# chlhnu/DOT-SOCP

Measured on AMD Instinct MI355X. Metric: ADMM iters/sec on NxNxT dot2d staggered grid at 1/2/4/8 MI355X, higher is better.
Workload: dtype f64

## Files before the change

### dot-socp_amd/csrc/fused.hip

```cpp
#include "device_utils.h"
#include "gather_tile.h"
#include "kernels.h"

#include <cstdlib>

namespace dotsocp {

template <int MODE, int XB, bool NT = false, bool GIN = false, bool GOUT = false>
__global__ void __launch_bounds__(64 * XB) k_cone_fused(Grid g, LoopCoef c, FusedArgs a) {
    static_assert(MODE == 1 || !(GIN || GOUT), "the gamma form exists between two MODE_B passes only");
    constexpr bool DUAL = (MODE >= 5);
    constexpr bool UPD = (MODE != 0 && MODE != 6);
    constexpr bool PROJ = (MODE < 2 || MODE >= 5);
    __shared__ double2 xch[2][XB][64];
    __shared__ double2 xchp[DUAL ? 2 : 1][DUAL ? XB : 1][DUAL ? 64 : 1];
    const int lane = threadIdx.x, xl = threadIdx.y;
    const BlockId blk = block_id(a.xcd != 0);
    const i64 y = (i64)blk.x * 64 + lane;
    const i64 x = (i64)blk.y * XB + xl;
    const bool inb = (y < g.ny) && (x < g.nx);
    const i64 yc = inb ? y : 0, xc = inb ? x : 0;
    const i64 t0 = ((i64)blk.z + a.z0) * a.TC;
    const i64 t1 = (t0 + a.TC < g.ncl) ? t0 + a.TC : g.ncl;
    const bool lastChunk = (t1 == g.ncl);
// ... 10 lines not shown
        const i64 ci = yc + g.py * xc;
        gc.p3 = a.carry_in[ci]; gc.p4 = a.carry_in[g.plane + ci];
        gc.p7 = a.carry_in[2 * g.plane + ci]; gc.p8 = a.carry_in[3 * g.plane + ci];
    }
    const i64 tstop = (GATHER && lastChunk) ? t1 + 1 : t1;
    for (i64 tl = tstart; tl < tstop; ++tl) {
        const bool hasCell = tl < g.ncl;
        const bool own = tl >= t0;
        double w[10], wp[10];
        if (hasCell) {
            const i64 i = yc + g.py * (xc + g.nx * tl);
            const EdgeQuad nxt = load_edges(g, a.q, yc, xc, tl + 1, c.sf);
            double b[10], v[10];
#pragma unroll
            for (int j = 0; j < 10; ++j) b[j] = ld_stream<NT>(a.beta_in + j * g.Nc + i);
            if (!GIN) apply_scale_ops(b, a.bops);
            build_z2(v, a.q[i], cur, nxt, c.s, c.dF);
            if constexpr (GIN) {
#pragma unroll
                for (int j = 0; j < 10; ++j) b[j] = mult_finish(b[j], v[j], c.tau);
                if (!GOUT && own && inb) {
#pragma unroll
                    for (int j = 0; j < 10; ++j) st_stream<NT>(a.beta_out + j * g.Nc + i, b[j]);
                }
            } else if constexpr (UPD) {
                const EdgeQuad nxto = load_edges(g, a.q_old, yc, xc, tl + 1, c.sf);
                double zo[10];
                build_z2(zo, a.q_old[i], curo, nxto, c.s, c.dF);
#pragma unroll
                for (int j = 0; j < 10; ++j) zo[j] = zo[j] - b[j];
                proj_row<10>(zo);
#pragma unroll
                for (int j = 0; j < 10; ++j) b[j] = mult_finish(mult_carry(b[j], zo[j], c.tau), v[j], c.tau);
                if (own && inb) {
                    if (MODE != 3 && !GOUT) {
#pragma unroll
                        for (int j = 0; j < 10; ++j) st_stream<NT>(a.beta_out + j * g.Nc + i, b[j]);
                    }
                    if (MODE == 2 || MODE == 3) {
#pragma unroll
                        for (int j = 0; j < 10; ++j) st_stream<NT>(a.z_out + j * g.Nc + i, zo[j]);
                    }
                }
                curo = nxto;
                if (MODE == 4) {
#pragma unroll
                    for (int j = 0; j < 10; ++j) w[j] = zo[j] + b[j];
                    if (own && inb) a.q2[i] = c.s * (w[9] - w[0]);
                }
            }
            cur = nxt;
            if (PROJ) {
                if (MODE == 5) {
                    const EdgeQuad nxt3 = load_edges(g, a.q3, yc, xc, tl + 1, c.sf);
                    build_z2(v, a.q3[i], cur3, nxt3, c.s, c.dF);
                    cur3 = nxt3;
                }
#pragma unroll
                for (int j = 0; j < 10; ++j) v[j] = v[j] - b[j];
                proj_row<10>(v);
                if (GOUT && own && inb) {
#pragma unroll
                    for (int j = 0; j < 10; ++j) st_stream<NT>(a.beta_out + j * g.Nc + i, mult_carry(b[j], v[j], c.tau));
                }
#pragma unroll
                for (int j = 0; j < 10; ++j) w[j] = v[j] + b[j];
// ... 106 lines not shown
```

### dot-socp_amd/csrc/kernels.h

```cpp
#pragma once
#include "common.h"
#include "defer.h"
#include "particle_block.h"

namespace dotsocp {

struct LoopCoef {
    double s;
    double sf;
    double dF;
    double at, ax, ay;
    double tau;
    double c1, c2;
    double dinv1, dinv2;
};

enum {
    S_Q2 = 0, S_Z2, S_APHI2, S_ALPHA2, S_BETA2, S_FBBETA2, S_PRIM1, S_PRIM2, S_DUAL1, S_DUAL2,
    S_COMPLEM, S_DOTCOMP, S_RHO2, S_RHOFQ2, S_MRHOB, S_M2, S_RHOB2, S_QALPHA, S_CPHI, S_PHI2,
    S_COUNT
};

struct KktCoef {
    double sigma;
// ... 15 lines not shown
        return true;
    }
};

int launch_proj_soc(double *out, const double *in, i64 M, i64 K, hipStream_t st);
int launch_bfd(const Grid &g, double *z, const double *q, double s, double dF, hipStream_t st);
int launch_bfd_conj(const Grid &g, double *q, const double *w, double s, hipStream_t st, const double *tail_bx = nullptr,
                    const double *tail_by = nullptr);
int launch_cone_proj(const Grid &g, const LoopCoef &c, const double *q, const double *beta, double *z,
                     hipStream_t st);
int launch_beta_update(const Grid &g, const LoopCoef &c, const double *q, const double *z, double *beta,
                       hipStream_t st);
int launch_gather_tail(const Grid &g, const double *z, const double *beta, double *tail_bx, double *tail_by,
                       hipStream_t st);

struct FusedGeom {
    int XB;
    i64 nyblk, nxblk;
    i64 TC, chunks;
    i64 sx_len, sy_len;
};
struct FusedArgs {
    const double *q_old;
    const double *q;
    const double *beta_in;
    double *beta_out;
    double *z_out;
    double *q2;
    double *sx, *sy;
    const double *q3;
    double *p2, *sxp, *syp;
    i64 TC;
    ScaleOps bops;
    int xcd;
    int z0;
    const double *carry_in;
    double *carry_out;
};
bool tile_xcd_remap(const Grid &g);
int fused_geometry(const Grid &g, FusedGeom &fg);
enum { CONE_GIN = 1, CONE_GOUT = 2 };
int launch_cone_fused(int mode, const Grid &g, const LoopCoef &c, const FusedGeom &fg, FusedArgs a,
                      hipStream_t st, i64 z0 = 0, i64 zcount = -1, int flavour = 0);
bool cone_split_enabled();

struct KktWork;
struct AccArgs {
    const double *q;
    const double *z_in, *beta_in;
    const double *z0, *beta0;
    double *z0_out, *beta0_out;
    double bdiv;
    KktCoef kk;
    const double *alpha_p, *weight;
    double *partials;
    int nostore;
    double *z_out, *beta_out;
    double *q2, *sx, *sy;
    i64 TC;
    double c1, c2, om_rho, rho;
};
struct AccCoef {
    double c1, c2, om_rho, rho;
    double om_c1, c1c2;
};
int launch_acc_cone(int mode, const Grid &g, const LoopCoef &c, const FusedGeom &fg, AccArgs a, hipStream_t st);
// ... 220 lines not shown
```

### dot-socp_amd/csrc/kkt.hip

```cpp
#include "device_utils.h"
#include "gather_tile.h"
#include "kernels.h"

#include <cstdlib>

namespace dotsocp {

struct WBeta {
    const double *b;
    i64 Nz;
    __device__ __forceinline__ double operator()(int j, i64 cell) const { return b[j * Nz + cell]; }
};

template <bool WEIGHTED, int PART, bool NODUAL = false>
__global__ void __launch_bounds__(TILE_Y *TILE_X) k_kkt(Grid g, LoopCoef c, KktCoef k, i64 chunk,
                                                         const double *__restrict__ phi, const double *__restrict__ q,
                                                         const double *__restrict__ alpha, const double *__restrict__ z,
                                                         const double *__restrict__ beta,
                                                         const double *__restrict__ cvec,
                                                         const double *__restrict__ weight,
                                                         KktHalo halo, double *__restrict__ partials,
                                                         double *__restrict__ resid) {
    const i64 y = (i64)blockIdx.x * TILE_Y + threadIdx.x;
    const i64 x = (i64)blockIdx.y * TILE_X + threadIdx.y;
// ... 122 lines not shown
                double tmp = (-c.ay) * phi[node];
                tmp += c.ay * phi[node + 1];
                const double q2b = NODUAL ? 0.0 : c.sf * gather_by(g, WB, y, x, tl, halo.btail_by);
                edge_sums(idx, tmp, q2b);
                const double rm = (rho_node(y, x, tl) + rho_node(y + 1, x, tl)) / 2.0;
                const double rb = k.dsD * (rm * q[idx]);
                const double m = k.kappa * (wgt(idx) * alpha[idx]);
                const double d = m - rb;
                S[S_MRHOB] += d * d;
                S[S_M2] += m * m;
                S[S_RHOB2] += rb * rb;
            }
        }
    }
    __shared__ double red[TILE_X][S_COUNT];
    const int lane = threadIdx.x;
#pragma unroll
    for (int i = 0; i < S_COUNT; ++i) {
        double v = S[i];
#pragma unroll
        for (int off = 32; off >= 1; off >>= 1) v += __shfl_down(v, off, 64);
        if (lane == 0) red[threadIdx.y][i] = v;
    }
    __syncthreads();
    if (threadIdx.y == 0 && lane < S_COUNT) {
        double v = red[0][lane];
#pragma unroll
        for (int wv = 1; wv < TILE_X; ++wv) v += red[wv][lane];
        const i64 b = blockIdx.x + (i64)gridDim.x * (blockIdx.y + (i64)gridDim.y * blockIdx.z);
        partials[b * S_COUNT + lane] = v;
    }
}

template <bool WEIGHTED, bool EDGES, bool NORMS = false, bool NT = false>
__global__ void __launch_bounds__(TILE_Y *TILE_X) k_kkt_cells(Grid g, LoopCoef c, KktCoef k, FusedArgs a,
                                                               const double *__restrict__ phi,
                                                               const double *__restrict__ alpha,
                                                               const double *__restrict__ weight,
                                                               double *__restrict__ partials) {
    __shared__ double2 xch[EDGES ? 2 : 1][EDGES ? TILE_X : 1][EDGES ? 64 : 1];
    const int lane = threadIdx.x, xl = threadIdx.y;
    const i64 y = (i64)blockIdx.x * TILE_Y + lane;
    const i64 x = (i64)blockIdx.y * TILE_X + xl;
    const bool inb = (y < g.ny) && (x < g.nx);
    const i64 yc = inb ? y : 0, xc = inb ? x : 0;
    const i64 t0 = (i64)blockIdx.z * a.TC;
    const i64 t1 = (t0 + a.TC < g.ncl) ? t0 + a.TC : g.ncl;
    const bool lastChunk = (t1 == g.ncl);
    const i64 tstart = (EDGES && t0 > 0) ? t0 - 1 : t0;
    const i64 tstop = (EDGES && lastChunk) ? t1 + 1 : t1;
    const i64 nxblk = gridDim.y, nyblk = gridDim.x;
    double S[S_COUNT];
#pragma unroll
    for (int i = 0; i < S_COUNT; ++i) S[i] = 0.0;
    auto wgt = [&](i64 idx) { return WEIGHTED ? weight[idx] : 1.0; };
    double p3 = 0.0, p4 = 0.0, p7 = 0.0, p8 = 0.0;
    int par = 0;
    if (inb || EDGES) {
        EdgeQuad cur = load_edges(g, a.q, yc, xc, tstart, c.sf);
        EdgeQuad curo = load_edges(g, a.q_old, yc, xc, tstart, c.sf);
        for (i64 tl = tstart; tl < tstop; ++tl) {
            const bool hasCell = tl < g.ncl;
            const bool own = (tl >= t0) && inb;
            double b[10];
            if (hasCell) {
                const i64 i = yc + g.py * (xc + g.nx * tl);
                const EdgeQuad nxt = load_edges(g, a.q, yc, xc, tl + 1, c.sf);
                const EdgeQuad nxto = load_edges(g, a.q_old, yc, xc, tl + 1, c.sf);
                const double q0 = a.q[i];
                double v[10], zo[10];
#pragma unroll
                for (int j = 0; j < 10; ++j) b[j] = ld_stream<NT>(a.beta_in + j * g.Nc + i);
                apply_scale_ops(b, a.bops);
                build_z2(v, q0, cur, nxt, c.s, c.dF);
                build_z2(zo, a.q_old[i], curo, nxto, c.s, c.dF);
#pragma unroll
                for (int j = 0; j < 10; ++j) zo[j] = zo[j] - b[j];
                proj_row<10>(zo);
                double zs = 0.0, bs = 0.0, rs = 0.0;
#pragma unroll
                for (int j = 0; j < 10; ++j) {
                    const double r = zo[j] - v[j];
                    b[j] = mult_finish(mult_carry(b[j], zo[j], c.tau), v[j], c.tau);
                    zs += zo[j] * zo[j];
                    bs += b[j] * b[j];
                    rs += r * r;
                }
                cur = nxt;
                curo = nxto;
                if (own && NORMS) {
                    S[S_Z2] += zs;
                    S[S_BETA2] += bs;
                }
                if (own && !NORMS) {
#pragma unroll
                    for (int j = 0; j < 10; ++j) st_stream<NT>(a.beta_out + j * g.Nc + i, b[j]);
                    auto xj = [&](int j) { return zo[j] - k.sigma * b[j]; };
                    const double n = sqrt(soc_norm2(xj, 10)), x0 = xj(0);
                    double cf = (x0 / n + 1.0) * 0.5;
                    cf = (cf > 1.0) ? 1.0 : cf;
                    cf = (cf < 0.0) ? 0.0 : cf;
                    const double p0 = (cf >= 1.0) ? x0 : cf * n;
                    double cs = (zo[0] - p0) * (zo[0] - p0);
#pragma unroll
                    for (int j = 1; j < 10; ++j) {
                        const double d = zo[j] - cf * xj(j);
                        cs += d * d;
                    }
                    S[S_Z2] += zs;
                    S[S_BETA2] += bs;
                    S[S_PRIM2] += rs;
                    S[S_COMPLEM] += cs;
                    const double w = wgt(i);
                    const double av = alpha[i];
                    const double rhoT = k.kappa * (w * av);
                    double sq = 0.0;
#pragma unroll
                    for (int j = 1; j < 9; ++j) {
                        const double e = k.dsE * v[j];
                        sq += e * e;
                    }
                    double rhoFq = rhoT + k.dsD * q0 + sq / 4.0;
                    rhoFq = (rhoFq < 0.0) ? 0.0 : rhoFq;
                    const double dd = rhoT - rhoFq;
                    S[S_DOTCOMP] += dd * dd;
                    S[S_RHO2] += rhoT * rhoT;
                    S[S_RHOFQ2] += rhoFq * rhoFq;
                    const double q2b = c.s * (b[9] - b[0]);
                    const double wa = w * av;
// ... 273 lines not shown
#undef KKT_ND
    DS_HIP(hipGetLastError());
    return 0;
}

int launch_kkt_bnd_dual(const Grid &g, const LoopCoef &c, const KktCoef &k, const FusedGeom &fg, const double *q,
                        const double *alpha, const double *weight, const double *q2, const double *sx, const double *sy,
                        const KktWork &w, hipStream_t st) {
    const i64 region = kkt_region_blocks(g);
    for (int dir = 0; dir < 2; ++dir) {
        const i64 len = dir == 0 ? g.ny : g.nx, lines = dir == 0 ? fg.nxblk : fg.nyblk;
        if (len <= 0 || lines <= 0) continue;
        dim3 gb((unsigned)((len + 255) / 256), (unsigned)lines, (unsigned)((g.ntl + BND_TC - 1) / BND_TC));
        double *pb = w.partials + (2 + dir) * region * S_COUNT;
#define BND(W, D) DS_KLAUNCH((k_kkt_bnd<W, D, true>), gb, dim3(256), 0, st, g, c, k, fg, q, alpha, weight, q2, sx, sy, pb)
        if (weight) { if (dir == 0) BND(true, 0); else BND(true, 1); }
        else { if (dir == 0) BND(false, 0); else BND(false, 1); }
#undef BND
        DS_HIP(hipGetLastError());
    }
    return 0;
}

int launch_kkt_cells_update(const Grid &g, const LoopCoef &c, const KktCoef &k, const FusedGeom &fg, FusedArgs a,
                            const double *phi, const double *alpha, const double *weight, const KktWork &w,
                            hipStream_t st, bool edges, const double *q_new) {
    if (g.Nz <= 0) return 0;
    const i64 region = kkt_region_blocks(g);
    a.TC = fg.TC;
    dim3 grid((unsigned)fg.nyblk, (unsigned)fg.nxblk, (unsigned)fg.chunks);
    double *part = w.partials + 1 * region * S_COUNT;
    const dim3 blk(TILE_Y, TILE_X);
    if (!edges) {
        if (weight) DS_KLAUNCH((k_kkt_cells<true, false>), grid, blk, 0, st, g, c, k, a, phi, alpha, weight, part);
        else DS_KLAUNCH((k_kkt_cells<false, false>), grid, blk, 0, st, g, c, k, a, phi, alpha, weight, part);
        DS_HIP(hipGetLastError());
        return 0;
    }
    const bool nt = stream_nt_enabled();
    if (weight) {
        if (nt) DS_KLAUNCH((k_kkt_cells<true, true, false, true>), grid, blk, 0, st, g, c, k, a, phi, alpha, weight, part);
        else DS_KLAUNCH((k_kkt_cells<true, true>), grid, blk, 0, st, g, c, k, a, phi, alpha, weight, part);
    } else {
        if (nt) DS_KLAUNCH((k_kkt_cells<false, true, false, true>), grid, blk, 0, st, g, c, k, a, phi, alpha, weight, part);
        else DS_KLAUNCH((k_kkt_cells<false, true>), grid, blk, 0, st, g, c, k, a, phi, alpha, weight, part);
    }
    DS_HIP(hipGetLastError());
    for (int dir = 0; dir < 2; ++dir) {
        const i64 len = dir == 0 ? g.ny : g.nx, lines = dir == 0 ? fg.nxblk : fg.nyblk;
        if (len <= 0 || lines <= 0) continue;
        dim3 gb((unsigned)((len + 255) / 256), (unsigned)lines, (unsigned)((g.ntl + BND_TC - 1) / BND_TC));
        double *pb = w.partials + (2 + dir) * region * S_COUNT;
#define BND(W, D) DS_KLAUNCH((k_kkt_bnd<W, D>), gb, dim3(256), 0, st, g, c, k, fg, q_new, alpha, weight, a.q2, a.sx, a.sy, pb)
        if (weight) { if (dir == 0) BND(true, 0); else BND(true, 1); }
        else { if (dir == 0) BND(false, 0); else BND(false, 1); }
#undef BND
        DS_HIP(hipGetLastError());
    }
    return 0;
}

int launch_norms(const Grid &g, const LoopCoef &c, const KktCoef &k, const FusedGeom &fg, FusedArgs a, const double *phi,
                 const double *alpha, const double *weight, const KktWork &w, hipStream_t st) {
    const i64 region = kkt_region_blocks(g);
    a.TC = fg.TC;
    if (g.Nz > 0) {
        dim3 grid((unsigned)fg.nyblk, (unsigned)fg.nxblk, (unsigned)fg.chunks);
        double *part = w.partials + 1 * region * S_COUNT;
        if (weight) DS_KLAUNCH((k_kkt_cells<true, false, true>), grid, dim3(TILE_Y, TILE_X), 0, st, g, c, k, a, phi, alpha, weight, part);
        else DS_KLAUNCH((k_kkt_cells<false, false, true>), grid, dim3(TILE_Y, TILE_X), 0, st, g, c, k, a, phi, alpha, weight, part);
    }
    struct R { const double *x; i64 n; int slot, reg; };
    const R rs[] = {{phi, g.Nphi, S_PHI2, 0},
// ... 29 lines not shown
```

### dot-socp_amd/csrc/schedule.h

```cpp
#pragma once

namespace dotsocp {

inline bool if_adjust_sigma(double iter, double last_iter) {
    const double passed = iter - last_iter;
    if (iter < 20 && passed >= 3) return true;
    if (iter < 50 && passed >= 6) return true;
    if (iter < 100 && passed >= 10) return true;
    if (iter < 200 && passed >= 15) return true;
    if (iter < 500 && passed >= 25) return true;
    return passed >= 40;
}
inline bool check_scheduled(long long it, double lastSigmaIt, long long maxit, bool stepByStep) {
    return stepByStep || if_adjust_sigma((double)it, lastSigmaIt) || it >= maxit;
}
inline bool norm_check_due(long long it, int rescale) { return rescale >= 3 && (it % 100) == 0; }
inline bool rescale_trigger(long long it, int rescale, double maxFeas, double relGap) {
    return (rescale == 1 && maxFeas < 2e-2 && it >= 10 && relGap < 5e-2) ||
           (rescale == 2 && maxFeas < 5e-3 && it >= 50 && relGap < 1e-2);
}
inline bool rescale_due(long long it, int rescale, double maxFeas, double relGap) {
    return norm_check_due(it, rescale) || rescale_trigger(it, rescale, maxFeas, relGap);
}

struct SchedState {
    long long it, maxit;
    double lastSigmaIt;
    bool checkStepByStep;
    int rescale;
    double maxFeas, relGap;
    long long run_left;
};
inline SchedState next_iteration(SchedState s) {
    s.it += 1;
    if (s.run_left > 0) s.run_left -= 1;
    return s;
}
inline bool cone_writes_beta(const SchedState &s) {
    return check_scheduled(s.it, s.lastSigmaIt, s.maxit, s.checkStepByStep) || (s.run_left >= 0 && s.run_left <= 1) ||
           rescale_due(s.it + 1, s.rescale, s.maxFeas, s.relGap);
}
enum { QCONE_NONE = 0, QCONE_STEADY = 1, QCONE_EXIT = 2 };
inline int qcone_form(const SchedState &s) {
    if (cone_writes_beta(s)) return QCONE_NONE;
    return cone_writes_beta(next_iteration(s)) ? QCONE_EXIT : QCONE_STEADY;
}
inline bool timeout_check_waits(bool gamma_left, bool early_pending) { return gamma_left || early_pending; }

struct StepIn {
    SchedState s;
    bool fused, deferred, cone_carry, kkt_fold;
    bool beta_gamma;
    bool timeout_pending;
    int early;
    bool qcone_eligible;
    bool inter;
    bool can_split_z, can_split_q;
};
struct StepPlan {
    bool adjust_sigma, kkt_due, fold, split_z, split_q;
    bool cone_launch;
    bool pass_gout;
    bool gamma_after;
    int qcone_candidate;
    bool error;
};

inline StepPlan plan_step(const StepIn &in) {
    StepPlan p{};
    const SchedState &s = in.s;
    p.adjust_sigma = if_adjust_sigma((double)s.it, s.lastSigmaIt);
    p.kkt_due = check_scheduled(s.it, s.lastSigmaIt, s.maxit, s.checkStepByStep) ||
                (in.timeout_pending && !timeout_check_waits(in.early == QCONE_STEADY, false));
    p.pass_gout = in.cone_carry && in.fused && in.deferred && !p.kkt_due && !cone_writes_beta(s);
    p.fold = p.kkt_due && in.kkt_fold && in.fused;
    p.split_z = in.inter && in.can_split_z;
    p.split_q = in.inter && in.can_split_q;
    p.cone_launch = (in.early == QCONE_NONE);
    p.error = !p.cone_launch && (p.split_z || !in.fused || !in.deferred || p.pass_gout != (in.early == QCONE_STEADY));
    if (p.error) return p;
    p.gamma_after = (p.cone_launch && in.deferred) ? p.pass_gout : in.beta_gamma;
    if (in.qcone_eligible && !p.fold && in.deferred && p.gamma_after) p.qcone_candidate = qcone_form(s);
    return p;
}

}
```

### dot-socp_amd/csrc/solver.h

```cpp
#pragma once
#include <chrono>
#include <functional>
#include <memory>
#include <string>
#include <type_traits>
#include <utility>
#include <vector>

#include "hostmem.h"
#include "kernels.h"
#include "schedule.h"

namespace dotsocp {

constexpr unsigned long long POISON_WORD = 0x7ff8bad0bad0bad0ull;
int guarded_malloc(void **p, size_t bytes, bool fp = false);
void guarded_free(void *p);
bool poison_enabled();
int poison_region(void *p, size_t bytes);
long long device_cache_release();
long long device_cache_held(int dev);
int canary_check(std::string *report);
bool canary_enabled();
bool stream_stress_enabled();
// ... 206 lines not shown
    bool checkPrimDualFeas = true;
    double time_limit = 3600.0;
    double sigma = 1.0, sigmaScale = 1.0;
    double cScale = 1.0, dScale = 1.0, D = 1.0, E = 1.0;
    double norm_c = 0.0, norm_d = 0.0;
    double h = 1.0;
    int rescale = 0, use_feasOrg = 0;
    double maxFeas = 0.0, relGap = 0.0, tol_feasOrg = 0.0;
    double lastSigmaIt = 0.0;
    i64 it = 0;
    LoopCoef lc{};
    std::vector<double> hist_kkt, hist_time, hist_iter, hist_gap;
    std::chrono::steady_clock::time_point t_begin;
    double elapsed_prev = 0.0;
    double elapsed_agreed = 0.0;
    bool deferred = false;
    bool z_valid = true;
    bool z_prev_ok = false;
    bool rhs_valid = false;
    bool cone_carry = true;
    bool beta_gamma = false;
    i64 run_left = -1;
    int qcone = -1;
    bool q_valid = true;
    int early_pass = QCONE_NONE;
    StepIn step_in() const;
    int need_q(const char *who) const;
    bool time_limit_passed() const;
    i64 timeout_at = -1;
    bool timeout_pending = false;
    int need_beta_form(const char *who) const;
    ScaleOps bops{0, 1.0, 1.0, 1.0, 1.0};
    ScaleOps zp_ops{0, 1.0, 1.0, 1.0, 1.0};
    int push_beta_op(double mul, double div);
    int flush_beta();
    ScaleOps aops{0, 1.0, 1.0, 1.0, 1.0};
    int flush_alpha();
    int sigma_scale_folded(double factor);
    FusedArgs pending_step_args(const Slab &s) const;
    double last_S[S_COUNT] = {0};
    double last_S_sigma = 1.0;
    i64 last_S_it = -1;
    bool norm_cache = true;
    bool kkt_fold = true;
    KktCoef kkt_coef() const;
    int clear_partials(Slab &s);
    int begin(const dotsocp_opts *o);
    int begin_method(const dotsocp_opts *o, int method, const dotsocp_acc_opts *acc);
    int run(i64 n_iters, i64 *done);
    int finish(dotsocp_result *res);
    int step(bool *brk);
    int rescale_block();
    int poisson_all(const PhiHooks *hooks = nullptr);
    int poisson_phi();
    int phase_phi(const PhiHooks *hooks = nullptr);
    int phase_z(const StepPlan &plan, int part);
    int phase_q(const StepPlan &plan, int part, int early = QCONE_NONE);
    int phase_mult();
    int materialise();
    int ensure_z();
    int kkt_sums(double *S, bool folded = false);
    int reduce_sums(double *S);
    int norms_light(double *S);
    int kkt_block(bool adjustSigmaYes, bool timed_out, bool *brk, bool folded = false);
    int scale_state(double a_mul, double a_div, double q_div, bool with_c);
    void update_coef();
    double elapsed() const;
    bool profiling = false;
    struct Pending { hipEvent_t a, b; int phase; };
    std::vector<Pending> pending;
    std::vector<hipEvent_t> event_pool;
    double phase_ms[PH_COUNT] = {0};
    i64 phase_launches[PH_COUNT] = {0};
    void prof_begin(int phase, bool on_z = false);
    void prof_end(int phase, bool on_z = false);
    int prof_flush();

    int method = DOTSOCP_METHOD_INPALM;
    i64 acc_restart = 100, acc_k = 0;
    double acc_rho = 2.0, acc_theta = 2.0;
    bool acc_halpern = true;
    bool acc_gather_valid = false;
    bool acc_swapped = false;
    bool acc_post = true;
    bool acc_light = false;
    double acc_factor = 1.0;
    int acc_alloc();
    int acc_begin(const dotsocp_acc_opts *acc);
    int acc_step(bool *brk);
    int acc_rescale_block();
    int acc_set_anchors();
    void acc_swap_state();
    int acc_on_sigma_factor(double factor);
    AccCoef acc_coef() const;
    bool palm_fast = true;
    bool palm_p_valid = false;
    int palm_begin();
// ... 18 lines not shown
```

### dot-socp_amd/csrc/solver.hip

```cpp
#include "solver.h"

#include <algorithm>
#include <cmath>
#include <cstring>

#include "comm.h"

namespace dotsocp {

void Solver::update_coef() {
    lc.s = E / D;
    lc.sf = edge_factor(lc.s);
    lc.dF = E / dScale;
    const double ht = 1.0 / (double)(nt - 1);
    lc.at = D * (1.0 / ht);
    lc.ax = (nx > 1) ? D * (1.0 / (1.0 / (double)(nx - 1))) : 0.0;
    lc.ay = (ny > 1) ? D * (1.0 / (1.0 / (double)(ny - 1))) : 0.0;
    lc.tau = opts.tau;
    const double tmp = (E / D) * (E / D);
    if (prob.weighted) { lc.c1 = 2.0 * tmp; lc.c2 = tmp; }
    else { lc.c1 = 1.0 + 2.0 * tmp; lc.c2 = 1.0 + tmp; }
    lc.dinv1 = 1.0 / lc.c1;
    lc.dinv2 = 1.0 / lc.c2;
}

int Solver::need_beta_form(const char *who) const {
    if (!beta_gamma) return 0;
    set_error("internal: %s met the gamma form of beta", who);
    return DOTSOCP_ESTATE;
}

int Solver::need_q(const char *who) const {
    if (q_valid) return 0;
    set_error("internal: %s met a q that was never stored", who);
    return DOTSOCP_ESTATE;
}

int Solver::flush_beta() {
    DS_CHECK(need_beta_form("flush_beta"));
    if (bops.empty()) return 0;
    FOR_SLABS(s) {
        DS_CHECK(launch_scale(s.beta, 10 * s.g.Nc, bops.mul, bops.div, s.st));
        if (bops.n > 1) DS_CHECK(launch_scale(s.beta, 10 * s.g.Nc, bops.mul2, bops.div2, s.st));
    }
    bops.clear();
    return 0;
}

int Solver::push_beta_op(double mul, double div) {
    if (bops.push(mul, div)) return 0;
    DS_CHECK(flush_beta());
    bops.push(mul, div);
    return 0;
}

FusedArgs Solver::pending_step_args(const Slab &s) const {
    FusedArgs a{};
    a.q_old = s.q_old;
    a.q = s.q;
    a.beta_in = s.beta;
    a.bops = bops;
    return a;
}

int Solver::clear_partials(Slab &s) {
    DS_HIP(ds_memset_async(s.kw.partials, 0, sizeof(double) * s.kw.maxBlocks * S_COUNT, s.st));
    return 0;
}

int Solver::flush_alpha() {
    if (aops.empty()) return 0;
    FOR_SLABS(s) DS_CHECK(launch_scale(s.alpha, s.g.NqAlloc, aops.mul, aops.div, s.st));
    aops.clear();
    return 0;
}

int Solver::sigma_scale_folded(double factor) {
    DS_CHECK(flush_alpha());
    DS_CHECK(ensure_halo());
    u0_made = false;
    DS_CHECK(push_beta_op(1.0, factor));
    if (multi()) {
        FOR_SLABS(s) DS_CHECK(launch_scale(s.alpha, s.g.NqAlloc, 1.0, factor, s.st));
    } else {
        aops.push(1.0, factor);
    }
    u0_fresh = false;
    FOR_SLABS(s) DS_CHECK(launch_rhs_sigma_fix(s.g, s.w0, s.w1, s.c, factor, s.st, c_ends_on && s.c_ends));
    return 0;
}

int Solver::scale_state(double a_mul, double a_div, double q_div, bool with_c) {
    DS_CHECK(need_beta_form("scale_state"));
    DS_CHECK(need_q("scale_state"));
    DS_CHECK(flush_alpha());
    if (begun) DS_CHECK(ensure_halo());
    u0_made = false;
    u0_fresh = false;
    rhs_valid = false;
    if (fused && begun) {
        DS_CHECK(push_beta_op(a_mul, a_div));
    }
    FOR_SLABS(s) {
        const Grid &g = s.g;
        if (with_c) DS_CHECK(launch_scale(s.c, g.Nphi, a_mul, a_div, s.st));
        if (!acc_light) DS_CHECK(launch_scale(s.alpha, g.NqAlloc, a_mul, a_div, s.st));
        if (!(fused && begun) && !acc_light) DS_CHECK(launch_scale(s.beta, 10 * g.Nc, a_mul, a_div, s.st));
        if (q_div != 1.0) {
            DS_CHECK(launch_scale(s.q, g.NqAlloc, 1.0, q_div, s.st));
            if (!(fused && begun) || z_valid) DS_CHECK(launch_scale(s.z, 10 * g.Nc, 1.0, q_div, s.st));
        }
    }
    if (q_div != 1.0 && fused && begun && !z_valid) z_prev_ok = false;
    return 0;
// ... 149 lines not shown
    }
    prof_begin(PH_RHS);
    if (!rhs_valid) {
        DS_CHECK(need_q("phase_phi"));
        DS_CHECK(flush_alpha());
        FOR_SLABS(s) DS_CHECK(launch_rhs(s.g, lc, s.q, s.alpha, s.c, s.weight, s.u0_prev, s.w0, s.st, c_ends_on && s.c_ends));
    } else if (multi()) {
        FOR_SLABS(s)
            if (!s.g.first) DS_CHECK(launch_rhs_fixup(s.g, lc, s.u0_prev, s.w0, s.st));
    }
    rhs_valid = false;
    prof_end(PH_RHS);
    prof_begin(PH_POISSON);
    DS_CHECK(poisson_all(hooks));
    prof_end(PH_POISSON);
    return 0;
}

static void part_chunks(int part, i64 C, i64 *z0, i64 *zc) {
    *z0 = (part == 2) ? C - 1 : 0;
    *zc = (part == 0) ? C : ((part == 1) ? C - 1 : 1);
}

int Solver::phase_z(const StepPlan &plan, int part) {
    DS_CHECK(need_q("phase_z"));
    if (part != 1) DS_CHECK(ensure_halo());
    if (!fused) {
        prof_begin(PH_PROJ);
        FOR_SLABS(s) DS_CHECK(launch_cone_proj(s.g, lc, s.q, s.beta, s.z, s.st));
        prof_end(PH_PROJ);
        return 0;
    }
    const bool gin = beta_gamma, gout = plan.pass_gout;
    if (gin && (!deferred || !bops.empty())) {
        set_error("internal: gamma form %s", deferred ? "with a pending scaling of beta" : "without a pending multiplier step");
        return DOTSOCP_ESTATE;
    }
    const int flavour = (gin ? CONE_GIN : 0) | (gout ? CONE_GOUT : 0);
    const int ph = deferred ? (gin ? PH_CONE_CARRY : PH_FUSED_B) : PH_FUSED_A;
    z_valid = false;
    z_prev_ok = false;
    prof_begin(ph);
    FOR_SLABS(s) {
        FusedArgs a{};
        a.q = s.q;
        a.q2 = s.q2;
        a.sx = s.sx;
        a.sy = s.sy;
        a.beta_in = s.beta;
        a.bops = bops;
        const i64 C = s.fg.chunks;
        i64 z0, zc;
        part_chunks(part, C, &z0, &zc);
        if (deferred) {
            a.q_old = s.q_old;
            a.beta_out = s.beta2;
        }
        const int mode = deferred ? 1 : 0;
        if (s.carry && C > 1) {
            for (i64 z = z0; z < z0 + zc; ++z) {
                a.carry_in = (z > 0) ? s.carry : nullptr;
                a.carry_out = (z + 1 < C) ? s.carry : nullptr;
                DS_CHECK(launch_cone_fused(mode, s.g, lc, s.fg, a, s.st, z, 1, flavour));
            }
        } else {
            DS_CHECK(launch_cone_fused(mode, s.g, lc, s.fg, a, s.st, z0, zc, flavour));
        }
        if (deferred && part != 1) std::swap(s.beta, s.beta2);
    }
    prof_end(ph);
    if (part == 1) return 0;
    if (deferred) {
        bops.clear();
        beta_gamma = gout;
    }
    return 0;
}

KktCoef Solver::kkt_coef() const {
    KktCoef k;
    k.sigma = sigma;
    k.kappa = sigma * cScale * D;
    k.dsD = dScale / D;
    k.dsE = dScale / E;
    return k;
}

int Solver::phase_q(const StepPlan &plan, int part, int early) {
    const bool kkt = plan.fold;
    if (!fused) DS_CHECK(flush_alpha());
    if (early != QCONE_NONE && (part != 0 || kkt || multi() || !fused || !deferred || !beta_gamma || !bops.empty())) {
        set_error("internal: early cone pass in a state it does not serve");
        return DOTSOCP_ESTATE;
    }
    const bool egout = (early == QCONE_STEADY);
    const int ph = (early != QCONE_NONE) ? PH_QCONE : PH_QSTEP;
    prof_begin(ph);
    FOR_SLABS(s) {
        hipStream_t st = s.st;
        if (early != QCONE_NONE && qcone != 2) {
            if (!s.sx2) {
                DS_CHECK(s.zalloc(&s.sx2, s.fg.sx_len));
                DS_CHECK(s.zalloc(&s.sy2, s.fg.sy_len));
            }
            QConeArgs a{};
            a.phi = s.phi; a.q2v = s.q2; a.sx = s.sx; a.sy = s.sy; a.cvec = s.c; a.alpha_in = s.alpha; a.gamma_in = s.beta;
            a.alpha_out = s.alpha2; a.rhs = s.w0; a.q_out = s.q_old; a.beta_out = s.beta2;
            a.q2_out = s.q; a.sx_out = s.sx2; a.sy_out = s.sy2;
            a.ap_on = aops.n; a.ap_mul = aops.mul; a.ap_div = aops.div;
            a.c_ends = (c_ends_on && s.c_ends) ? 1 : 0;
            DS_CHECK(launch_qcone(s.g, lc, s.fg, a, egout, st));
            s.rotate_after_qcone();
        } else if (!fused) {
            DS_CHECK(launch_qstep(s.g, lc, s.phi, s.z, s.beta, s.weight, s.tail_bx, s.tail_by, s.q, s.alpha, s.st));
        } else {
            i64 z0, zc;
            part_chunks(part, qstep_rhs_chunks(s.g, s.fg), &z0, &zc);
            QStepExtra ex{};
            ex.aops = aops;
            ex.c_ends = (c_ends_on && s.c_ends) ? 1 : 0;
            if (multi() && !s.g.last && part != 1) ex.u0_tail = s.send_plane;
            if (kkt) {
                const KktCoef k = kkt_coef();
                ex.partials = kkt_qstep_partials(s.g, s.kw);
// ... 27 lines not shown
    u0_made = multi() && fused;
    if (fused) aops.clear();
    rhs_valid = fused;
    if (multi() && fused && comm_z && cone_split_enabled()) halo_pending = true;
    else DS_CHECK(exchange_q_halo(true));
    return 0;
}

int Solver::phase_mult() {
    if (fused) {
        deferred = true;
        return 0;
    }
    prof_begin(PH_BETA);
    FOR_SLABS(s) DS_CHECK(launch_beta_update(s.g, lc, s.q, s.z, s.beta, s.st));
    prof_end(PH_BETA);
    return 0;
}

int Solver::materialise() {
    if (!fused || !deferred) return 0;
    DS_CHECK(need_beta_form("materialise"));
    DS_CHECK(need_q("materialise"));
    DS_CHECK(ensure_halo());
    prof_begin(PH_MATERIALISE);
    FOR_SLABS(s) {
        FusedArgs a = pending_step_args(s);
        a.beta_out = s.beta;
        a.z_out = s.z;
        DS_CHECK(launch_cone_fused(2, s.g, lc, s.fg, a, s.st));
    }
    prof_end(PH_MATERIALISE);
    bops.clear();
    deferred = false;
    z_valid = true;
    return 0;
}

int Solver::ensure_z() {
    if (!fused || z_valid) return 0;
    DS_CHECK(need_beta_form("ensure_z"));
    DS_CHECK(need_q("ensure_z"));
    if (deferred) return materialise();
    if (!z_prev_ok) {
        set_error("internal: z cannot be regenerated");
        return DOTSOCP_ESTATE;
    }
    DS_CHECK(ensure_halo());
    prof_begin(PH_MATERIALISE);
    FOR_SLABS(s) {
        FusedArgs a{};
        a.q_old = s.q_old;
        a.q = s.q;
        a.beta_in = s.beta2;
        a.z_out = s.z;
        a.bops = zp_ops;
        DS_CHECK(launch_cone_fused(3, s.g, lc, s.fg, a, s.st));
    }
    prof_end(PH_MATERIALISE);
    z_valid = true;
    return 0;
}

int Solver::kkt_sums(double *S, bool folded) {
    DS_CHECK(need_beta_form("kkt_sums"));
    DS_CHECK(need_q("kkt_sums"));
    DS_CHECK(ensure_halo());
    const KktCoef k = kkt_coef();
    if (method == DOTSOCP_METHOD_ACCADMM && folded) {
        FOR_SLABS(s) DS_CHECK(launch_kkt_nodual(s.g, lc, k, s.phi, s.q, s.alpha, s.c, s.weight, s.kw, s.st));
        return reduce_sums(S);
    }
    if (!folded) {
        DS_CHECK(flush_alpha());
        FOR_SLABS(s) DS_CHECK(clear_partials(s));
    }
    int rest = folded ? 0 : (1 | 4 | 8);
    if (fused && deferred) {
        FOR_SLABS(s) {
            FusedArgs a = pending_step_args(s);
            a.beta_out = s.beta2;
            if (folded) { a.q2 = s.q2; a.sx = s.sx; a.sy = s.sy; }
            DS_CHECK(launch_kkt_cells_update(s.g, lc, k, s.fg, a, s.phi, s.alpha, s.weight, s.kw, s.st, folded, s.q));
            std::swap(s.beta, s.beta2);
        }
        zp_ops = bops;
        bops.clear();
        deferred = false;
        z_valid = false;
        z_prev_ok = true;
    } else {
        if (folded) { set_error("internal: folded KKT sums without a pending multiplier step"); return DOTSOCP_ESTATE; }
        DS_CHECK(ensure_z());
        DS_CHECK(flush_beta());
        rest |= 2;
    }
    if (multi()) {
        const i64 plane = slabs[0].g.plane;
        u0_made = false;
        FOR_SLABS(s)
            if (!s.g.last)
                DS_CHECK(launch_kkt_tail(s.g, s.alpha, s.beta, s.weight, s.send_plane, s.send_plane2, s.send_bx, s.send_by,
                                         s.st));
        DS_CHECK(group_begin());
        DS_CHECK(shift(+1, [](Slab &s) { return s.send_plane; }, [](Slab &s) { return s.a0_prev; }, plane));
        DS_CHECK(shift(+1, [](Slab &s) { return s.send_plane2; }, [](Slab &s) { return s.a0w_prev; }, plane));
        DS_CHECK(shift(+1, [](Slab &s) { return s.send_bx; }, [](Slab &s) { return s.btail_bx; }, slabs[0].g.bxLayer));
        DS_CHECK(shift(+1, [](Slab &s) { return s.send_by; }, [](Slab &s) { return s.btail_by; }, slabs[0].g.byLayer));
        DS_CHECK(group_end());
    }
    FOR_SLABS(s) {
        KktHalo halo{s.a0_prev, s.a0w_prev, s.btail_bx, s.btail_by};
        if (rest) DS_CHECK(launch_kkt(s.g, lc, k, s.phi, s.q, s.alpha, s.z, s.beta, s.c, s.weight, halo, s.kw, rest, s.st));
        if (folded && !s.g.first)
            DS_CHECK(launch_kkt(s.g, lc, k, s.phi, s.q, s.alpha, s.z, s.beta, s.c, s.weight, halo, s.kw, 1 | 4 | 8, s.st, true,
                                s.w1));
    }
    return reduce_sums(S);
}

// ... 70 lines not shown
    if (norm_check_due(it, rescale)) {
        DS_CHECK(norms(normPhis, normAlps));
        const double ratio = std::max(normAlps, normPhis) / std::min(normAlps, normPhis);
        if (ratio > 1.2) scaleYes = true;
    }
    if (!(rescale_trigger(it, rescale, maxFeas, relGap) || scaleYes)) return 0;
    if (!scaleYes) DS_CHECK(norms(normPhis, normAlps));
    DS_CHECK(materialise());
    const double dScale2 = normPhis, cScale2 = normAlps;
    sigma = sigma * (cScale2 / dScale2);
    norm_c = norm_c / cScale2;
    if (!prob.weighted) norm_d = norm_d / dScale2;
    DS_CHECK(scale_state(dScale2, cScale2 * cScale2, dScale2, true));
    if (method == DOTSOCP_METHOD_PALM) {
        FOR_SLABS(s) DS_CHECK(launch_scale(s.phi, s.g.NphiAlloc, 1.0, dScale2, s.st));
    }
    dScale = dScale2 * dScale;
    cScale = cScale2 * cScale;
    sigmaScale = sigmaScale * (cScale2 / dScale2);
    update_coef();
    rescale += 1;
    return 0;
}

bool Solver::time_limit_passed() const {
    return timeout_pending || (remote() ? false : (elapsed() > time_limit || (timeout_at > 0 && it >= timeout_at)));
}

StepIn Solver::step_in() const {
    StepIn in{};
    in.s = SchedState{it, opts.maxit, lastSigmaIt, opts.ifCheckStepByStep != 0, rescale, maxFeas, relGap, run_left};
    in.fused = fused; in.deferred = deferred; in.cone_carry = cone_carry; in.kkt_fold = kkt_fold;
    in.beta_gamma = beta_gamma; in.timeout_pending = timeout_pending; in.early = early_pass;
    const Slab &s0 = slabs[0];
    in.qcone_eligible = qcone != 0 && fused && !multi() && !prob.weighted && method == DOTSOCP_METHOD_INPALM &&
                        s0.g.ncl >= 1 && s0.fg.XB == 4 &&
                        (qcone > 0 || s0.fg.nyblk * s0.fg.nxblk >= 2048);
    in.inter = comm_z && multi() && fused;
    in.can_split_z = in.can_split_q = in.inter && cone_split_enabled();
    for (auto &s : slabs) {
        in.can_split_z = in.can_split_z && s.fg.chunks >= 2;
        in.can_split_q = in.can_split_q && qstep_rhs_chunks(s.g, s.fg) >= 2;
    }
    return in;
}

static const double kUpdateRule[11][2] = {
    {1.1, 1.10}, {1.2, 1.15}, {1.5, 1.20}, {2, 1.26}, {2.5, 1.28}, {3.33, 1.32},
    {5, 1.35}, {10, 1.40}, {20, 1.60}, {40, 1.80}, {50, 2.00}};

static double get_factor(double xi) {
    double factor = 1.0;
    for (int i = 0; i < 11; ++i) {
        if (xi >= kUpdateRule[i][0]) factor = kUpdateRule[i][1];
        else break;
    }
    return factor;
}

static void adjust_lagrangian_param(double &sigma, double xi, double &factor) {
    factor = 1.0;
    if (xi >= 1) factor = get_factor(xi);
    else if (xi < 1) factor = 1.0 / get_factor(1.0 / xi);
    if (factor != 1.0) {
        const double old = sigma;
        sigma = std::max(std::min(sigma * factor, 1e3), 1e-3);
        factor = sigma / old;
    }
}

int Solver::kkt_block(bool adjustSigmaYes, bool timed_out, bool *brk, bool folded) {
    double S[S_COUNT + 1];
    prof_begin(PH_KKT);
    DS_CHECK(kkt_sums(S, folded));
    prof_end(PH_KKT);
    if (remote()) timed_out = elapsed_agreed > time_limit;
    for (int i = 0; i < S_COUNT; ++i) last_S[i] = S[i];
    last_S_sigma = sigma;
    last_S_it = it;
    const double sh = sqrt(h);
    auto nrm = [&](int i) { return sh * sqrt(S[i]); };
    const double norm_q = nrm(S_Q2), norm_z = nrm(S_Z2), norm_Aphi = nrm(S_APHI2);
    const double norm_alpha = sigma * nrm(S_ALPHA2), norm_beta = sigma * nrm(S_BETA2);
    const double norm_FBbeta = sigma * nrm(S_FBBETA2);
    const double primFea1 = nrm(S_PRIM1), primFea2 = nrm(S_PRIM2);
    const double dualFea1 = sigma * nrm(S_DUAL1), dualFea2 = sigma * nrm(S_DUAL2);
    const double complem = nrm(S_COMPLEM);
    const double dotcomplem = nrm(S_DOTCOMP), normRho = nrm(S_RHO2), norm_rhoFq = nrm(S_RHOFQ2);
    const double mRhoB = nrm(S_MRHOB), normM = nrm(S_M2), normRhoB = nrm(S_RHOB2);
    const double kc = 1.0;
    const double den2 = prob.weighted ? (norm_q + norm_z) : norm_d;
    double org[7], res[5];
    org[0] = primFea1 / (kc * D / dScale + norm_Aphi + norm_q);
    org[1] = primFea2 / (kc * E / dScale + den2);
    org[2] = dualFea1 / (kc / cScale + norm_c);
    org[3] = complem / (kc * E / dScale + norm_z + norm_beta);
    org[4] = dualFea2 / (kc / cScale / D + norm_FBbeta + norm_alpha);
    org[5] = dotcomplem / (kc + normRho + norm_rhoFq);
    org[6] = mRhoB / (kc + normM + normRhoB);
    res[0] = primFea1 / (kc + norm_Aphi + norm_q);
    res[1] = primFea2 / (kc + den2);
    res[2] = dualFea1 / (kc + norm_c);
    res[3] = complem / (kc + norm_z + norm_beta);
    res[4] = dualFea2 / (kc + norm_FBbeta + norm_alpha);
    const double priVal = (sigma * cScale * dScale * h) * S[S_QALPHA];
    const double dualVal = (sigma * cScale * dScale * h) * S[S_CPHI];
    const double pdGap = fabs(priVal - dualVal) / (1 + fabs(priVal) + fabs(dualVal));
// ... 62 lines not shown
        PhiHooks hooks;
        hooks.fill = [&]() -> int {
            if (plan.split_z) DS_CHECK(phase_z(plan, 2));
            return make_tails();
        };
        hooks.behind = [&]() -> int { return async_comm([&]() { return send_tails(); }, EV_JOIN); };
        DS_CHECK(phase_phi(&hooks));
    } else {
        DS_CHECK(phase_phi());
        if (plan.cone_launch) DS_CHECK(phase_z(plan, 0));
    }
    if (plan.fold) {
        FOR_SLABS(s) DS_CHECK(clear_partials(s));
    }
    if (in.inter) {
        DS_CHECK(async_comm([&]() { return send_phi_head(); }, EV_HALO));
        DS_CHECK(comm_wait(EV_JOIN));
        if (plan.split_q) DS_CHECK(phase_q(plan, 1));
        DS_CHECK(comm_wait(EV_HALO));
        DS_CHECK(phase_q(plan, plan.split_q ? 2 : 0));
    } else {
        DS_CHECK(ship_tails());
        const bool early_ok = plan.qcone_candidate != QCONE_NONE && !time_limit_passed();
        DS_CHECK(phase_q(plan, 0, early_ok ? plan.qcone_candidate : QCONE_NONE));
    }
    DS_CHECK(phase_mult());
    const bool timed_out = time_limit_passed();
    timeout_pending = false;
    if (timed_out && timeout_check_waits(beta_gamma, early_pass != QCONE_NONE)) {
        timeout_pending = true;
        return 0;
    }
    if (plan.kkt_due || timed_out)
        DS_CHECK(kkt_block(plan.adjust_sigma, timed_out, brk, plan.fold));
    return 0;
}

int Solver::run(i64 n_iters, i64 *done) {
    if (!begun || finished) { set_error("run() needs begin() and must precede finish()"); return DOTSOCP_ESTATE; }
    cur_dev = -1;
    DS_CHECK(use_dev(device));
    struct DeferScope {
        DeferCtx *ctx;
        int err = 0;
        explicit DeferScope(DeferCtx *c) : ctx(c) { if (ctx) { g_defer = ctx; ctx->begin(); } }
        int close() { if (ctx) { err = ctx->end(); g_defer = nullptr; ctx = nullptr; } return err; }
        ~DeferScope() { (void)close(); }
    } scope(defer.get());
    i64 n = 0;
    while (it < opts.maxit && !stopped) {
        if (n_iters >= 0 && n >= n_iters) break;
        bool brk = false;
        run_left = (n_iters >= 0) ? n_iters - n : -1;
        DS_CHECK(step(&brk));
        if (brk) stopped = true;
        ++n;
    }
    DS_CHECK(need_beta_form("the end of run()"));
    DS_CHECK(need_q("the end of run()"));
    if (early_pass != QCONE_NONE) { set_error("internal: an early cone pass is pending at the end of run()"); return DOTSOCP_ESTATE; }
    DS_CHECK(ensure_halo());
    DS_CHECK(sync_all());
    DS_CHECK(prof_flush());
    if (const int derr = scope.close()) {
        set_error("a HIP call issued by a slab thread failed: %s", hipGetErrorString((hipError_t)derr));
        return DOTSOCP_EHIP;
    }
// ... 100 lines not shown
```

### dot-socp_amd/csrc/solver_slabs.hip

```cpp
#include "solver.h"

#include <algorithm>
#include <cmath>
#include <cstring>

#include "comm.h"

namespace dotsocp {

thread_local std::string g_last_error;

static int make_eig_table(double **dev, i64 n, i64 len = 0);

void set_error(const char *fmt, ...) {
    char buf[1024];
    va_list ap;
    va_start(ap, fmt);
    vsnprintf(buf, sizeof buf, fmt, ap);
    va_end(ap);
    g_last_error = buf;
}

int Solver::use_dev(int d) {
    if (cur_dev == d) return 0;
// ... 124 lines not shown
}

int Solver::init(const dotsocp_problem *p, int dev, int nslabs, bool multi_dev) {
    DS_ARG(p != nullptr, "prob is NULL");
    DS_ARG(p->dim == 1 || p->dim == 2, "prob.dim must be 1 or 2");
    DS_ARG(p->nt >= 2 && p->nx >= 1, "grid too small");
    prob = *p;
    device = dev;
    if (p->dim == 1) { ny = p->nx; nx = 1; } else { ny = p->ny; nx = p->nx; }
    nt = p->nt;
    DS_ARG(ny >= 1 && nx >= 1, "grid too small");
    DS_ARG(nslabs >= 1 && nslabs <= nt / 2, "nslabs must be in [1, nt/2]");
    DS_CHECK(dct_length_check(ny)); DS_CHECK(dct_length_check(nx)); DS_CHECK(dct_length_check(nt));
    if (const char *e = getenv("DOTSOCP_FUSED")) fused = (atoi(e) != 0);
    if (nslabs > 1 && !fused) {
        set_error("time slabs need the fused dataflow (unset DOTSOCP_FUSED=0)");
        return DOTSOCP_EINVAL;
    }
    int ndev = 0;
    if (hipGetDeviceCount(&ndev) != hipSuccess || ndev <= 0) {
        set_error("no HIP device available (libdotsocp has no CPU fallback)");
        return DOTSOCP_ENODEVICE;
    }
    DS_ARG(dev >= 0 && dev < ndev, "device ordinal out of range");
    ndev_visible = ndev;
    multi_device = multi_dev && nslabs > 1;
    cur_dev = -1;
    DS_CHECK(use_dev(dev));
    DS_HIP(hipStreamCreateWithFlags(&stream, hipStreamNonBlocking));
    DS_CHECK(make_second_stream(&stream_z));
    overlap = nslabs > 1;
    if (const char *e = getenv("DOTSOCP_OVERLAP")) overlap = (atoi(e) != 0);
    if (const char *e = getenv("DOTSOCP_KKT_FOLD")) kkt_fold = (atoi(e) != 0);
    if (const char *e = getenv("DOTSOCP_NORM_CACHE")) norm_cache = (atoi(e) != 0);
    tri_tsolve = tsolve_tri_allowed();
    DS_HIP(hipHostMalloc((void **)&h_sums, sizeof(double) * (S_COUNT + 1)));
    DS_CHECK(dmalloc(&d_red, S_COUNT + 1));
    if (!res_for(dev)) return DOTSOCP_EHIP;
    world = nslabs;
    rank = 0;
    return 0;
}

int Solver::ensure_alloc() {
    if (!slabs.empty()) return 0;
    DS_CHECK(alloc_slabs(remote() ? rank : 0, remote() ? 1 : world));
    DS_CHECK(sync_all());
    return 0;
}

i64 Solver::column_pad() const { return (ny * nx >= 4096) ? 48 : 0; }

i64 Solver::row_pitch() const {
    static const bool on = !(getenv("DOTSOCP_PITCH") && atoi(getenv("DOTSOCP_PITCH")) == 0);
    if (!on || ny <= 16) return ny;
    if (ny % 16 == 0) {
        const char *e = getenv("DOTSOCP_PITCH2");
        const bool on2 = !(e && atoi(e) == 0);
        return (on2 && ny >= 512 && ny % 256 == 0) ? ny + 16 : ny;
    }
    return (ny + 15) / 16 * 16;
}

int Solver::alloc_slabs(int first, int count) {
    free_slabs();
    peer_ok = true;
// ... 157 lines not shown
```

Before: 95.88.

## Keep the multiplier step pending across folded KKT checks to skip a beta store

When a folded KKT check runs on a single device with the deferred fused dataflow, the KKT cell pass now computes the updated beta for its norms without writing beta_out, and leaves the multiplier step pending for the next cone pass. A new pending scale-op set (pops) carries the sigma rescale of beta forward so the next fused cone pass applies it after the multiplier update. This removes a full 10-component f64 beta store and its later reload on KKT iterations, at the cost of more scheduling state, new error paths and recomputing the update in the following pass. It is on by default (kkt_pending=1) and gated on unweighted problems with qcone eligibility.

```diff
diff --git a/dot-socp_amd/csrc/fused.hip b/dot-socp_amd/csrc/fused.hip
--- a/dot-socp_amd/csrc/fused.hip
+++ b/dot-socp_amd/csrc/fused.hip
@@ -66,6 +66,7 @@
                 proj_row<10>(zo);
 #pragma unroll
                 for (int j = 0; j < 10; ++j) b[j] = mult_finish(mult_carry(b[j], zo[j], c.tau), v[j], c.tau);
+                if constexpr (MODE == 1 || MODE == 2) apply_scale_ops(b, a.pops);
                 if (own && inb) {
                     if (MODE != 3 && !GOUT) {
 #pragma unroll
diff --git a/dot-socp_amd/csrc/kernels.h b/dot-socp_amd/csrc/kernels.h
--- a/dot-socp_amd/csrc/kernels.h
+++ b/dot-socp_amd/csrc/kernels.h
@@ -71,6 +71,7 @@
     double *p2, *sxp, *syp;
     i64 TC;
     ScaleOps bops;
+    ScaleOps pops;
     int xcd;
     int z0;
     const double *carry_in;
diff --git a/dot-socp_amd/csrc/kkt.hip b/dot-socp_amd/csrc/kkt.hip
--- a/dot-socp_amd/csrc/kkt.hip
+++ b/dot-socp_amd/csrc/kkt.hip
@@ -178,7 +178,7 @@
     }
 }
 
-template <bool WEIGHTED, bool EDGES, bool NORMS = false, bool NT = false>
+template <bool WEIGHTED, bool EDGES, bool NORMS = false, bool NT = false, bool KEEP = false>
 __global__ void __launch_bounds__(TILE_Y *TILE_X) k_kkt_cells(Grid g, LoopCoef c, KktCoef k, FusedArgs a,
                                                                const double *__restrict__ phi,
                                                                const double *__restrict__ alpha,
@@ -229,9 +229,11 @@
                     const double r = zo[j] - v[j];
                     b[j] = mult_finish(mult_carry(b[j], zo[j], c.tau), v[j], c.tau);
                     zs += zo[j] * zo[j];
-                    bs += b[j] * b[j];
                     rs += r * r;
                 }
+                apply_scale_ops(b, a.pops);
+#pragma unroll
+                for (int j = 0; j < 10; ++j) bs += b[j] * b[j];
                 cur = nxt;
                 curo = nxto;
                 if (own && NORMS) {
@@ -239,8 +241,10 @@
                     S[S_BETA2] += bs;
                 }
                 if (own && !NORMS) {
-#pragma unroll
-                    for (int j = 0; j < 10; ++j) st_stream<NT>(a.beta_out + j * g.Nc + i, b[j]);
+                    if constexpr (!KEEP) {
+#pragma unroll
+                        for (int j = 0; j < 10; ++j) st_stream<NT>(a.beta_out + j * g.Nc + i, b[j]);
+                    }
                     auto xj = [&](int j) { return zo[j] - k.sigma * b[j]; };
                     const double n = sqrt(soc_norm2(xj, 10)), x0 = xj(0);
                     double cf = (x0 / n + 1.0) * 0.5;
@@ -580,13 +584,18 @@
     double *part = w.partials + 1 * region * S_COUNT;
     const dim3 blk(TILE_Y, TILE_X);
     if (!edges) {
+        if (!a.beta_out) { set_error("internal: the unfolded cell pass stores beta"); return DOTSOCP_ESTATE; }
         if (weight) DS_KLAUNCH((k_kkt_cells<true, false>), grid, blk, 0, st, g, c, k, a, phi, alpha, weight, part);
         else DS_KLAUNCH((k_kkt_cells<false, false>), grid, blk, 0, st, g, c, k, a, phi, alpha, weight, part);
         DS_HIP(hipGetLastError());
         return 0;
     }
     const bool nt = stream_nt_enabled();
-    if (weight) {
+    if (!a.beta_out) {
+        if (weight) { set_error("internal: the no-store cell pass serves unweighted problems only"); return DOTSOCP_ESTATE; }
+        if (nt) DS_KLAUNCH((k_kkt_cells<false, true, false, true, true>), grid, blk, 0, st, g, c, k, a, phi, alpha, weight, part);
+        else DS_KLAUNCH((k_kkt_cells<false, true, false, false, true>), grid, blk, 0, st, g, c, k, a, phi, alpha, weight, part);
+    } else if (weight) {
         if (nt) DS_KLAUNCH((k_kkt_cells<true, true, false, true>), grid, blk, 0, st, g, c, k, a, phi, alpha, weight, part);
         else DS_KLAUNCH((k_kkt_cells<true, true>), grid, blk, 0, st, g, c, k, a, phi, alpha, weight, part);
     } else {
diff --git a/dot-socp_amd/csrc/schedule.h b/dot-socp_amd/csrc/schedule.h
--- a/dot-socp_amd/csrc/schedule.h
+++ b/dot-socp_amd/csrc/schedule.h
@@ -19,6 +19,7 @@
     return (rescale == 1 && maxFeas < 2e-2 && it >= 10 && relGap < 5e-2) ||
            (rescale == 2 && maxFeas < 5e-3 && it >= 50 && relGap < 1e-2);
 }
+inline bool rescale_armed(long long it, int rescale) { return (rescale == 1 && it >= 10) || (rescale == 2 && it >= 50); }
 inline bool rescale_due(long long it, int rescale, double maxFeas, double relGap) {
     return norm_check_due(it, rescale) || rescale_trigger(it, rescale, maxFeas, relGap);
 }
@@ -56,6 +57,7 @@
     bool qcone_eligible;
     bool inter;
     bool can_split_z, can_split_q;
+    int kkt_pending;
 };
 struct StepPlan {
     bool adjust_sigma, kkt_due, fold, split_z, split_q;
@@ -64,6 +66,7 @@
     bool gamma_after;
     int qcone_candidate;
     bool error;
+    bool keep_pending;
 };
 
 inline StepPlan plan_step(const StepIn &in) {
@@ -81,6 +84,13 @@
     if (p.error) return p;
     p.gamma_after = (p.cone_launch && in.deferred) ? p.pass_gout : in.beta_gamma;
     if (in.qcone_eligible && !p.fold && in.deferred && p.gamma_after) p.qcone_candidate = qcone_form(s);
+    if (in.kkt_pending && in.qcone_eligible && in.cone_carry && p.fold && !in.timeout_pending &&
+        check_scheduled(s.it, s.lastSigmaIt, s.maxit, s.checkStepByStep) && s.it < s.maxit && !(s.run_left >= 0 && s.run_left <= 1) &&
+        (in.kkt_pending >= 2 || !rescale_armed(s.it + 1, s.rescale))) {
+        SchedState nx = next_iteration(s);
+        if (p.adjust_sigma) nx.lastSigmaIt = (double)s.it;
+        p.keep_pending = in.kkt_pending >= 2 || !cone_writes_beta(nx);
+    }
     return p;
 }
 
diff --git a/dot-socp_amd/csrc/solver.h b/dot-socp_amd/csrc/solver.h
--- a/dot-socp_amd/csrc/solver.h
+++ b/dot-socp_amd/csrc/solver.h
@@ -262,6 +262,7 @@
     int need_beta_form(const char *who) const;
     ScaleOps bops{0, 1.0, 1.0, 1.0, 1.0};
     ScaleOps zp_ops{0, 1.0, 1.0, 1.0, 1.0};
+    ScaleOps pops{0, 1.0, 1.0, 1.0, 1.0};
     int push_beta_op(double mul, double div);
     int flush_beta();
     ScaleOps aops{0, 1.0, 1.0, 1.0, 1.0};
@@ -273,6 +274,7 @@
     i64 last_S_it = -1;
     bool norm_cache = true;
     bool kkt_fold = true;
+    int kkt_pending = 1;
     KktCoef kkt_coef() const;
     int clear_partials(Slab &s);
     int begin(const dotsocp_opts *o);
@@ -289,10 +291,10 @@
     int phase_mult();
     int materialise();
     int ensure_z();
-    int kkt_sums(double *S, bool folded = false);
+    int kkt_sums(double *S, bool folded = false, bool keep = false);
     int reduce_sums(double *S);
     int norms_light(double *S);
-    int kkt_block(bool adjustSigmaYes, bool timed_out, bool *brk, bool folded = false);
+    int kkt_block(bool adjustSigmaYes, bool timed_out, bool *brk, bool folded = false, bool keep = false);
     int scale_state(double a_mul, double a_div, double q_div, bool with_c);
     void update_coef();
     double elapsed() const;
diff --git a/dot-socp_amd/csrc/solver.hip b/dot-socp_amd/csrc/solver.hip
--- a/dot-socp_amd/csrc/solver.hip
+++ b/dot-socp_amd/csrc/solver.hip
@@ -48,6 +48,7 @@
 }
 
 int Solver::push_beta_op(double mul, double div) {
+    if (!pops.empty()) { set_error("internal: a scaling of beta in front of a pending multiplier step that carries one"); return DOTSOCP_ESTATE; }
     if (bops.push(mul, div)) return 0;
     DS_CHECK(flush_beta());
     bops.push(mul, div);
@@ -60,6 +61,7 @@
     a.q = s.q;
     a.beta_in = s.beta;
     a.bops = bops;
+    a.pops = pops;
     return a;
 }
 
@@ -79,7 +81,11 @@
     DS_CHECK(flush_alpha());
     DS_CHECK(ensure_halo());
     u0_made = false;
-    DS_CHECK(push_beta_op(1.0, factor));
+    if (deferred) {
+        if (!pops.push(1.0, factor)) { set_error("internal: two sigma updates behind one pending multiplier step"); return DOTSOCP_ESTATE; }
+    } else {
+        DS_CHECK(push_beta_op(1.0, factor));
+    }
     if (multi()) {
         FOR_SLABS(s) DS_CHECK(launch_scale(s.alpha, s.g.NqAlloc, 1.0, factor, s.st));
     } else {
@@ -295,7 +301,7 @@
         return 0;
     }
     const bool gin = beta_gamma, gout = plan.pass_gout;
-    if (gin && (!deferred || !bops.empty())) {
+    if (gin && (!deferred || !bops.empty() || !pops.empty())) {
         set_error("internal: gamma form %s", deferred ? "with a pending scaling of beta" : "without a pending multiplier step");
         return DOTSOCP_ESTATE;
     }
@@ -312,6 +318,7 @@
         a.sy = s.sy;
         a.beta_in = s.beta;
         a.bops = bops;
+        if (deferred) a.pops = pops;
         const i64 C = s.fg.chunks;
         i64 z0, zc;
         part_chunks(part, C, &z0, &zc);
@@ -335,6 +342,7 @@
     if (part == 1) return 0;
     if (deferred) {
         bops.clear();
+        pops.clear();
         beta_gamma = gout;
     }
     return 0;
@@ -352,7 +360,7 @@
 int Solver::phase_q(const StepPlan &plan, int part, int early) {
     const bool kkt = plan.fold;
     if (!fused) DS_CHECK(flush_alpha());
-    if (early != QCONE_NONE && (part != 0 || kkt || multi() || !fused || !deferred || !beta_gamma || !bops.empty())) {
+    if (early != QCONE_NONE && (part != 0 || kkt || multi() || !fused || !deferred || !beta_gamma || !bops.empty() || !pops.empty())) {
         set_error("internal: early cone pass in a state it does not serve");
         return DOTSOCP_ESTATE;
     }
@@ -446,6 +454,7 @@
     }
     prof_end(PH_MATERIALISE);
     bops.clear();
+    pops.clear();
     deferred = false;
     z_valid = true;
     return 0;
@@ -476,7 +485,7 @@
     return 0;
 }
 
-int Solver::kkt_sums(double *S, bool folded) {
+int Solver::kkt_sums(double *S, bool folded, bool keep) {
     DS_CHECK(need_beta_form("kkt_sums"));
     DS_CHECK(need_q("kkt_sums"));
     DS_CHECK(ensure_halo());
@@ -490,7 +499,14 @@
         FOR_SLABS(s) DS_CHECK(clear_partials(s));
     }
     int rest = folded ? 0 : (1 | 4 | 8);
-    if (fused && deferred) {
+    if (keep) {
+        if (!(folded && fused && deferred && !multi())) { set_error("internal: a KKT check cannot leave this multiplier step pending"); return DOTSOCP_ESTATE; }
+        FOR_SLABS(s) {
+            FusedArgs a = pending_step_args(s);
+            a.q2 = s.q2; a.sx = s.sx; a.sy = s.sy;
+            DS_CHECK(launch_kkt_cells_update(s.g, lc, k, s.fg, a, s.phi, s.alpha, s.weight, s.kw, s.st, true, s.q));
+        }
+    } else if (fused && deferred) {
         FOR_SLABS(s) {
             FusedArgs a = pending_step_args(s);
             a.beta_out = s.beta2;
@@ -500,6 +516,7 @@
         }
         zp_ops = bops;
         bops.clear();
+        pops.clear();
         deferred = false;
         z_valid = false;
         z_prev_ok = true;
@@ -636,6 +653,7 @@
     in.s = SchedState{it, opts.maxit, lastSigmaIt, opts.ifCheckStepByStep != 0, rescale, maxFeas, relGap, run_left};
     in.fused = fused; in.deferred = deferred; in.cone_carry = cone_carry; in.kkt_fold = kkt_fold;
     in.beta_gamma = beta_gamma; in.timeout_pending = timeout_pending; in.early = early_pass;
+    in.kkt_pending = kkt_pending;
     const Slab &s0 = slabs[0];
     in.qcone_eligible = qcone != 0 && fused && !multi() && !prob.weighted && method == DOTSOCP_METHOD_INPALM &&
                         s0.g.ncl >= 1 && s0.fg.XB == 4 &&
@@ -673,10 +691,10 @@
     }
 }
 
-int Solver::kkt_block(bool adjustSigmaYes, bool timed_out, bool *brk, bool folded) {
+int Solver::kkt_block(bool adjustSigmaYes, bool timed_out, bool *brk, bool folded, bool keep) {
     double S[S_COUNT + 1];
     prof_begin(PH_KKT);
-    DS_CHECK(kkt_sums(S, folded));
+    DS_CHECK(kkt_sums(S, folded, keep));
     prof_end(PH_KKT);
     if (remote()) timed_out = elapsed_agreed > time_limit;
     for (int i = 0; i < S_COUNT; ++i) last_S[i] = S[i];
@@ -805,7 +823,7 @@
         return 0;
     }
     if (plan.kkt_due || timed_out)
-        DS_CHECK(kkt_block(plan.adjust_sigma, timed_out, brk, plan.fold));
+        DS_CHECK(kkt_block(plan.adjust_sigma, timed_out, brk, plan.fold, plan.keep_pending && !timed_out));
     return 0;
 }
 
diff --git a/dot-socp_amd/csrc/solver_slabs.hip b/dot-socp_amd/csrc/solver_slabs.hip
--- a/dot-socp_amd/csrc/solver_slabs.hip
+++ b/dot-socp_amd/csrc/solver_slabs.hip
@@ -180,6 +180,7 @@
     overlap = nslabs > 1;
     if (const char *e = getenv("DOTSOCP_OVERLAP")) overlap = (atoi(e) != 0);
     if (const char *e = getenv("DOTSOCP_KKT_FOLD")) kkt_fold = (atoi(e) != 0);
+    if (const char *e = getenv("DOTSOCP_KKT_PENDING")) kkt_pending = atoi(e) < 0 ? 0 : (atoi(e) > 2 ? 2 : atoi(e));
     if (const char *e = getenv("DOTSOCP_NORM_CACHE")) norm_cache = (atoi(e) != 0);
     tri_tsolve = tsolve_tri_allowed();
     DS_HIP(hipHostMalloc((void **)&h_sums, sizeof(double) * (S_COUNT + 1)));
```

Result: no change. 95.84 (-0.0%).
